# AU-Master-Thesis/magics

Hardware: AMD Instinct MI355X
Metric: GBP iterations/sec (whole node), N robots x K horizon (higher is better)
Workload: dtype f64

## Files before the change

### magics_amd/csrc/mgx_dev.h

```cpp
#pragma once
#include <cstdint>

namespace mgx {

constexpr int SNAP_W = 24;

struct BlobLayout {
    int K, E1;
    __host__ __device__ constexpr BlobLayout(int k) : K(k), E1(4 * k - 6 + 1) {}
    __host__ __device__ constexpr int prior() const { return 0; }
    __host__ __device__ constexpr int bel() const { return 20 * K; }
    __host__ __device__ constexpr int cov() const { return 40 * K; }
    __host__ __device__ constexpr int mu() const { return 56 * K; }
    __host__ __device__ constexpr int fv() const { return 60 * K; }
    __host__ __device__ constexpr int valid() const { return 60 * K + 20 * E1; }
    __host__ __device__ constexpr int inout_words() const { return 16 * K + 4 * K + 20 * E1 + K; }
    __host__ __device__ constexpr int words() const { return 61 * K + 20 * E1; }
};

struct IrEdgeRec {
    int32_t src_var;
    int32_t src_robot;
    uint32_t created;
    int32_t dst;
// ... 183 lines not shown

constexpr int MAX_SEGS = 32;

struct LingerPlan {
    uint32_t n, has_upd;
    uint32_t ext[MAX_SEGS / 4], n_int[MAX_SEGS / 4];
    double upd_max_speed, upd_delta_t;
    unsigned long long number;
};
constexpr int LINGER_PLAN_DWORDS = (int)(sizeof(LingerPlan) / 4);
constexpr unsigned LINGER_SLOT_HEAD = 128u, LINGER_UPD_BYTES = 48u;
static_assert(LINGER_PLAN_DWORDS == 24, "eight chunks of three dwords");
struct LingerBox {
    unsigned long long posted;
    unsigned long long close_req;
    unsigned long long taken;
    unsigned long long reserved;
    unsigned long long closed;
    unsigned long long pad[3];
    LingerPlan plan[2];
};

struct SweepRan {
    int32_t variant = 0;
    int32_t ir_mode = -1;
};

struct SegPlan {
    int32_t n;
    uint8_t ext[MAX_SEGS];
    uint8_t n_int[MAX_SEGS];
    unsigned long long flag_base;
    long long timeout_ticks;
    unsigned long long launch_seq;
    long long census_ticks;
    unsigned long long agree_seq;
    long long linger_ticks;
    const LingerBox *linger_box;
    const double *linger_upd;
    unsigned long long linger_upd_stride;
    unsigned char *linger_dev;
    unsigned long long linger_dev_stride;
    unsigned long long *linger_go;
};
constexpr unsigned RESIDENT_GO = 1u, RESIDENT_ABORT = 2u;

constexpr int AGREE_LOOK = 0, AGREE_SIGN_IN = 1, AGREE_ABORT = 2;
constexpr int AGREE_HISTORY = 6;
constexpr unsigned AGREE_LOST = 3u;
__device__ inline unsigned agree_on_launch(unsigned long long *word, unsigned long long L, unsigned n_ranks, int action) {
    constexpr unsigned long long HMASK = (1ull << (2 * AGREE_HISTORY)) - 1ull;
    unsigned long long declined = 0ull;
    for (int i = 0; i < AGREE_HISTORY; i++) declined |= (unsigned long long)RESIDENT_ABORT << (2 * i);
    unsigned long long cur = __hip_atomic_load(word, __ATOMIC_RELAXED, __HIP_MEMORY_SCOPE_SYSTEM);
    for (;;) {
        const unsigned long long cl = cur >> 28, hist = (cur >> 16) & HMASK;
        const unsigned st = (unsigned)(cur >> 14) & 3u, cnt = (unsigned)cur & 0x3fffu;
        if (cl == L && st) return st;
        if (cl > L) {
            const unsigned long long back = cl - L;
            if (back > (unsigned long long)AGREE_HISTORY) return AGREE_LOST;
            const unsigned was = (unsigned)(hist >> (2 * (back - 1ull))) & 3u;
            return was ? was : AGREE_LOST;
        }
        if (action == AGREE_LOOK) return 0u;
        unsigned long long h = hist;
// ... 23 lines not shown
```

### magics_amd/csrc/mgx_sweep.h

```cpp
#pragma once
#include <hip/hip_runtime.h>

#include "gbp_math.h"
#include "mgx_dev.h"

namespace mgx {

constexpr int SWEEP_BLOCK = 128;
enum { ROLE_DYN = 0, ROLE_UV = 1 };
#ifndef MGX_WIDE
#define MGX_WIDE 0
#endif
template <int KT, bool PERSIST>
constexpr int sweep_waves() { return (MGX_WIDE && PERSIST && KT > 0 && 4 * KT <= 64) ? 4 : 2; }
template <int KT, bool PERSIST>
constexpr int sweep_threads() { return 64 * sweep_waves<KT, PERSIST>(); }

__device__ __forceinline__ void ld_soa4(const double *base, int stride, int item, double (&o)[4]) {
#pragma unroll
    for (int c = 0; c < 4; c++) o[c] = base[(size_t)c * stride + item];
}
__device__ __forceinline__ void ld_soa16(const double *base, int stride, int item, double (&o)[16]) {
#pragma unroll
    for (int c = 0; c < 16; c++) o[c] = base[(size_t)c * stride + item];
// ... 412 lines not shown
        const int a2 = 2 * slot, b2 = 2 * (1 - slot);
        const int it = r * (K - 1) + f;
#pragma unroll
        for (int i = 0; i < 2; i++)
#pragma unroll
            for (int j = 0; j < 2; j++) {
                paa[i * 2 + j] = w.dyn_m[(size_t)((a2 + i) * 4 + (a2 + j)) * w.ND + it];
                pab[i * 2 + j] = w.dyn_m[(size_t)((a2 + i) * 4 + (b2 + j)) * w.ND + it];
                pba[i * 2 + j] = w.dyn_m[(size_t)((b2 + i) * 4 + (a2 + j)) * w.ND + it];
                pbb[i * 2 + j] = w.dyn_m[(size_t)((b2 + i) * 4 + (b2 + j)) * w.ND + it];
            }
    };
    if (is_dyn) {
        const int f = lane % (K - 1), slot = lane / (K - 1);
        if (!PERSIST) load_dyn_potential(maa, mab, mba, mbb);
        dyn_other_var = f + 1 - slot;
        dyn_other_edge = (1 - slot) * (K - 1) + f;
    }
    const bool obs_rows = (4 * (K - 2) <= 64) && !(w.enable & 8u);
    const int uvar = (is_trk ? lane - (K - 2) : lane) + 1;
    const int uedge = n_dyn + lane;
    int trk_rec = 0;
    float trk_lp[2] = {0.f, 0.f};
    double trk_lv = 0.0;
    const int trk_item = r * (K - 2) + (uvar - 1);
    if (is_trk) {
        trk_rec = w.trk_record[trk_item];
        trk_lp[0] = w.trk_last_pos[trk_item];
        trk_lp[1] = w.trk_last_pos[(size_t)w.NT + trk_item];
        trk_lv = w.trk_last_val[trk_item];
    }

    const bool do_extf = !PERSIST && HAS_IR && (ext_mask & PH_EXT_FACTOR) && radio && ir_on;
    bool pf_on = false, pf_present = false;
    MGX_EDGE_REGS(pf_er);
    double pf_bmu[4] = {0.0, 0.0, 0.0, 0.0}, pf_rec[SNAP_W];
#pragma unroll
    for (int c = 0; c < SNAP_W; c++) pf_rec[c] = 0.0;
    uint8_t pf_gate = 0;
    int pf_dst = 0;
    const int n_in = (PERSIST && K > 1) ? ne / (K - 1) : 0;
    auto edge_of_lane = [&](int q) __attribute__((always_inline)) {
        if (!PERSIST) return q;
        const int c = q / (K - 1);
        return (q - c * (K - 1)) * n_in + c;
    };
    int my_j = (HAS_IR && tid < ne) ? edge_of_lane(tid) : 0;
    if (HAS_IR && tid < ne) pf_gate = w.ir_gate[ie0 + my_j];
    if (do_extf && tid < ne) {
        MGX_EDGE_LOAD(pf_er, &w.ir_rec[ie0 + my_j]);
        pf_dst = pf_er_dst;
        ld_soa4(w.ir_bmu, w.NI, ie0 + my_j, pf_bmu);
    }
    if (PERSIST && tid < ne) {
        MGX_EDGE_LOAD(pf_er, &w.ir_rec[ie0 + my_j]);
        pf_dst = pf_er_dst;
    }
    auto quad_gather = [&](auto fetch, unsigned ro_mine, double (&out)[SNAP_W]) __attribute__((always_inline)) {
        v4u32 R[4][3];
#pragma unroll
        for (int s4 = 0; s4 < 4; s4++) {
            unsigned rb;
            if (s4 == 0) rb = (unsigned)__builtin_amdgcn_mov_dpp((int)ro_mine, 0x00, 0xf, 0xf, true);
            else if (s4 == 1) rb = (unsigned)__builtin_amdgcn_mov_dpp((int)ro_mine, 0x55, 0xf, 0xf, true);
            else if (s4 == 2) rb = (unsigned)__builtin_amdgcn_mov_dpp((int)ro_mine, 0xAA, 0xf, 0xf, true);
            else rb = (unsigned)__builtin_amdgcn_mov_dpp((int)ro_mine, 0xFF, 0xf, 0xf, true);
#pragma unroll
            for (int t3 = 0; t3 < 3; t3++) R[s4][t3] = fetch(rb + 64u * t3 + 16u * (unsigned)(lane & 3));
        }
#pragma unroll
        for (int t3 = 0; t3 < 3; t3++) {
            unsigned dw[4][4];
#pragma unroll
            for (int wd = 0; wd < 4; wd++) {
                unsigned x[4] = {R[0][t3][wd], R[1][t3][wd], R[2][t3][wd], R[3][t3][wd]};
                quad_transpose4(x, lane);
#pragma unroll
                for (int v = 0; v < 4; v++) dw[wd][v] = x[v];
            }
#pragma unroll
            for (int v = 0; v < 4; v++) {
                out[2 * (4 * t3 + v)] = __hiloint2double((int)dw[1][v], (int)dw[0][v]);
                out[2 * (4 * t3 + v) + 1] = __hiloint2double((int)dw[3][v], (int)dw[2][v]);
            }
        }
    };
    auto fetch_plain = [&](unsigned off) __attribute__((always_inline)) {
        return *reinterpret_cast<const v4u32 *>(reinterpret_cast<const char *>(w.snap[w.cur]) + off);
    };
    uint32_t r_epoch = 0;
    int r_irp[3] = {0, 0, 0};
    if (tid < K) {
        r_epoch = w.snap_epoch[w.cur][v0 + tid];
        if (HAS_IR) {
            r_irp[0] = w.ir_var_ptr[v0 + tid];
            r_irp[1] = w.ir_var_mid[v0 + tid];
            r_irp[2] = w.ir_var_ptr[v0 + tid + 1];
        }
    }
    double u_rec[4] = {0.0, 0.0, 0.0, 0.0}, u_bel = 0.0;
    if (w.upd) {
#pragma unroll
        for (int c = 0; c < 4; c++) u_rec[c] = w.upd[(size_t)r * 4 + c];
        if (lane < 20 && role < 2) u_bel = blob[L.bel() + lane * K + (role == 0 ? K - 1 : 0)];
    }
    const bool recompute = (PERSIST ? plan.ext[0] != 0 : (ext_mask & PH_EXT_FACTOR) != 0) && radio && ir_on;
    double r_ir[6] = {0.0, 0.0, 0.0, 0.0, 0.0, 0.0};
    bool r_ir_on = false;

    auto chain_second_link = [&]() {
        if (STAGE_IR && tid < ne && !(recompute && pf_gate == 1)) {
            const size_t e = (size_t)(ie0 + my_j);
            r_ir_on = true;
            r_ir[0] = w.ir_fv_eta[0 * (size_t)w.NI + e];
            r_ir[1] = w.ir_fv_eta[1 * (size_t)w.NI + e];
            r_ir[2] = w.ir_fv_lam[0 * (size_t)w.NI + e];
            r_ir[3] = w.ir_fv_lam[1 * (size_t)w.NI + e];
            r_ir[4] = w.ir_fv_lam[4 * (size_t)w.NI + e];
            r_ir[5] = w.ir_fv_lam[5 * (size_t)w.NI + e];
        }
        if (do_extf) {
            pf_on = tid < ne && pf_gate == 1;
            if (pf_on) pf_present = w.snap_epoch[w.cur][pf_er_src_var] > pf_er_created;
            quad_gather(fetch_plain, pf_on ? (unsigned)pf_er_src_var * (unsigned)(SNAP_W * sizeof(double)) : 0u, pf_rec);
        }
    };
    unsigned long long early_decision = 0ull;
    {
        const double *src = w.snap[w.cur] + (size_t)v0 * SNAP_W;
        if constexpr (KT > 0) {
            StageRegs<20 * KT, NT> r_prior;
            StageRegs<BlobLayout(KT).inout_words() - 16 * KT, NT> r_io;
            constexpr int IT = (SNAP_W * KT + NT - 1) / NT;
            double r_snap[IT];
            r_prior.load(blob + L.prior(), tid);
            r_io.load(blob + L.mu(), tid);
#pragma unroll
            for (int it = 0; it < IT; it++) {
                const int t = tid + it * NT;
                r_snap[it] = (t < SNAP_W * K) ? src[t] : 0.0;
            }
            chain_second_link();
            if (census && BIG && tid == 0) early_decision = __hip_atomic_load(cold().decision, __ATOMIC_RELAXED, __HIP_MEMORY_SCOPE_AGENT);
            r_prior.store(s_prior, tid);
            r_io.store(s_mu, tid);
#pragma unroll
            for (int it = 0; it < IT; it++) {
                const int t = tid + it * NT;
                if (t < SNAP_W * K) s_snap[(t % SNAP_W) * K + (t / SNAP_W)] = r_snap[it];
            }
        } else {
            copy_words(s_prior, blob + L.prior(), 20 * K, tid, NT);
            chain_second_link();
            if (census && BIG && tid == 0) early_decision = __hip_atomic_load(cold().decision, __ATOMIC_RELAXED, __HIP_MEMORY_SCOPE_AGENT);
            copy_words(s_mu, blob + L.mu(), L.inout_words() - 16 * K, tid, NT);
            for (int t = tid; t < SNAP_W * K; t += NT) s_snap[(t % SNAP_W) * K + (t / SNAP_W)] = src[t];
// ... 41 lines not shown
                v = __hip_atomic_load(cold().decision, __ATOMIC_RELAXED, __HIP_MEMORY_SCOPE_AGENT);
                if ((v >> 2) != seq && wall_clock64() - t0 > 4 * cold_plan().census_ticks) {
                    if (SHARD && cold_plan().agree_seq != 0ull) {
                        const unsigned a = agree_on_launch(cold().agree, cold_plan().agree_seq, (unsigned)cold().n_ranks, AGREE_ABORT);
                        if (a == RESIDENT_GO) continue;
                        if (a == AGREE_LOST) __hip_atomic_store(cold().sweep_err, cold_plan().agree_seq, __ATOMIC_RELAXED, __HIP_MEMORY_SCOPE_SYSTEM);
                    }
                    if (__hip_atomic_compare_exchange_strong(cold().decision, &v, seq * 4ull + RESIDENT_ABORT, __ATOMIC_RELAXED, __ATOMIC_RELAXED,
                                                             __HIP_MEMORY_SCOPE_AGENT)) {
                        __hip_atomic_store(cold().decision_host, seq * 4ull + RESIDENT_ABORT, __ATOMIC_RELAXED, __HIP_MEMORY_SCOPE_SYSTEM);
                        v = seq * 4ull + RESIDENT_ABORT;
                    }
                }
            }
            abort_launch = (v & 3ull) == RESIDENT_ABORT ? 1 : 0;
        }
        return __syncthreads_or(abort_launch) != 0;
    };
    if (census && CENSUS_EARLY && census_says_abort(early_decision)) return;
    if (PLDS && w.upd) {
        if (tid < 4) s_urec[tid] = tid == 0 ? u_rec[0] : (tid == 1 ? u_rec[1] : (tid == 2 ? u_rec[2] : u_rec[3]));
        if (lane < 20 && role < 2) s_tmp[4 * K + role * 20 + lane] = u_bel;
        __syncthreads();
    }
    uint32_t my_epoch = 0u;
    STAMP(t_staged);

    const int VL = w.R_local * K;
    const unsigned xrec_bytes = PERSIST ? (unsigned)VL * (unsigned)XREC_BYTES : 0u;
    const __amdgpu_buffer_rsrc_t rs_x = sc1_rsrc(PERSIST ? w.xrec[0] : nullptr, 2u * xrec_bytes);
    constexpr unsigned GHOST_BIT = 0x80000000u;
    const unsigned gx_bytes = SHARD ? (unsigned)(w.V - VL) * (unsigned)XREC_BYTES : 0u;
    const __amdgpu_buffer_rsrc_t rs_gx = sc1_rsrc(SHARD ? w.gxrec[0] : nullptr, 2u * gx_bytes);
    auto gather_records = [&](auto fetch, bool mine, unsigned off_mine, uint32_t seq, double (&out)[SNAP_W], uint32_t &deliveries) __attribute__((always_inline)) {
        v4u32 R[XREC_CHUNKS];
        const unsigned cstride = 16u * (unsigned)K;
#pragma unroll
        for (int ch = 0; ch < XREC_CHUNKS; ch++) R[ch] = v4u32{0u, 0u, 0u, 0u};
        const bool remote = SHARD && (off_mine & GHOST_BIT) != 0u;
        const bool any_remote = SHARD && __ballot(remote) != 0ull;
        if (mine) {
#pragma unroll
            for (int ch = 0; ch < XREC_CHUNKS; ch++) R[ch] = fetch(off_mine + (unsigned)ch * cstride);
        }
        if constexpr (SHARD) {
            if (any_remote) {
#pragma unroll
                for (int ch = 0; ch < XREC_CHUNKS; ch++) R[ch].w ^= remote ? xrec_mix(R[ch].x, R[ch].y, R[ch].z) : 0u;
            }
        }
        auto word_of = [&](const v4u32 &c) __attribute__((always_inline)) { return c.w; };
        long long t0 = 0;
        for (unsigned spins = 0;; spins++) {
            bool missing = false;
#pragma unroll
            for (int ch = 0; ch < XREC_CHUNKS; ch++) missing = missing || word_of(R[ch]) != seq;
            missing = missing && mine;
            if (__ballot(missing) == 0ull) break;
#ifdef MGX_POLL_SLEEP
            __builtin_amdgcn_s_sleep(MGX_POLL_SLEEP);
#else
            __builtin_amdgcn_s_sleep(32);
#endif
            if (spins == 0u) t0 = wall_clock64();
            if ((spins & 31u) == 31u) {
                bool stop = __hip_atomic_load(cold().sweep_abort, __ATOMIC_RELAXED, __HIP_MEMORY_SCOPE_AGENT) != 0ull;
                if (!stop && wall_clock64() - t0 > cold_plan().timeout_ticks) {
                    __hip_atomic_store(cold().sweep_abort, (unsigned long long)seq, __ATOMIC_RELAXED, __HIP_MEMORY_SCOPE_AGENT);
                    __hip_atomic_store(cold().sweep_err, (unsigned long long)seq, __ATOMIC_RELAXED, __HIP_MEMORY_SCOPE_SYSTEM);
                    stop = true;
                }
                if (__ballot(stop) != 0ull) break;
            }
            if (missing) {
                unsigned again = 0u;
#pragma unroll
                for (int ch = 0; ch < XREC_CHUNKS; ch++)
                    if (word_of(R[ch]) != seq) { again |= 1u << ch; R[ch] = fetch(off_mine + (unsigned)ch * cstride); }
                if constexpr (SHARD) {
                    if (remote) {
#pragma unroll
                        for (int ch = 0; ch < XREC_CHUNKS; ch++)
                            if ((again >> ch) & 1u) R[ch].w ^= xrec_mix(R[ch].x, R[ch].y, R[ch].z);
                    }
                }
            }
        }
        auto D = [&](int n) __attribute__((always_inline)) { return R[n / 3][n % 3]; };
#pragma unroll
        for (int n = 0; n < 22; n++) out[n] = __hiloint2double((int)D(2 * n + 1), (int)D(2 * n));
        out[22] = 0.0;
        out[23] = 0.0;
        deliveries = D(XREC_EPOCH_DWORD);
#ifdef MGX_XREC_CHECKSUM
        if (mine) {
            unsigned x = 0u;
#pragma unroll
            for (int n = 0; n < XREC_PAYLOAD_DWORDS; n++) x ^= D(n);
            const unsigned o = off_mine & 0x7fffffffu, rob = o / ((unsigned)K * (unsigned)XREC_BYTES);
            const unsigned want_id = rob * 64u + (o - rob * (unsigned)K * (unsigned)XREC_BYTES) / 16u;
            if (x != R[15].x || R[15].y != want_id)
                __hip_atomic_store(cold().sweep_err, 0xBAD0000000000000ull | ((unsigned long long)(R[15].y & 0xfffffu) << 28) | ((unsigned long long)(want_id & 0xfffffu) << 8) | (seq & 0xffu),
                                   __ATOMIC_RELAXED, __HIP_MEMORY_SCOPE_SYSTEM);
        }
#endif
    };
    double *s_xmu = s_tmp;
    bool have_xmu = false;
#ifdef MGX_STAMPS
    unsigned long long q_arrive = 0ull, t_edges0 = 0ull;
    unsigned long long *tl = (PERSIST && w.dbg) ? w.dbg + (size_t)(w.R_local + 4) * 48 + (size_t)r * 64 : nullptr;
#define TLSTAMP(kk, what) do { if (tl && role == ROLE_UV && lane == 0 && (kk) >= 0 && (kk) < 16) tl[(kk) * 4 + (what)] = __builtin_amdgcn_s_memrealtime(); } while (0)
#else
#define TLSTAMP(kk, what)
#endif
    auto external_factor_sweep = [&](int k, int kg, bool store_fv) __attribute__((always_inline)) {
        const int buf = PERSIST ? ((w.cur + kg) & 1) : w.cur;
#ifdef MGX_STAMPS
        t_edges0 = __builtin_readcyclecounter();
#endif
        if (radio && ir_on) {
            auto fetch_xrec = [&](unsigned off) __attribute__((always_inline)) {
                if constexpr (SHARD) {
                    if (off & GHOST_BIT) return ld16_system_raw(rs_gx, off & ~GHOST_BIT, buf ? gx_bytes : 0u);
                }
                return ld16_agent_raw(rs_x, off, buf ? xrec_bytes : 0u);
            };
            const uint32_t want_seq = xrec_seq(plan.flag_base + (unsigned long long)kg);
            for (int j0 = 0; j0 < ne; j0 += NT) {
                const int q = j0 + tid;
                const int j = j0 == 0 ? my_j : (q < ne ? edge_of_lane(q) : 0);
                const int e = ie0 + j;
                MGX_EDGE_REGS(er);
                double ao_eta[4], ao_lam[16], a_mu[4], b_mu[4];
                bool a_present;
                double grec[SNAP_W];
                uint32_t grec_deliveries = 0u;
                bool mine = false;
                if (PERSIST || j0 > 0) {
                    if (j0 == 0) {
                        mine = tid < ne && pf_gate == 1;
                        if (mine) MGX_EDGE_COPY(er, pf_er);
                    } else if (j0 > 0 && q < ne && w.ir_gate[e] == 1) {
                        mine = true;
                        MGX_EDGE_LOAD(er, &w.ir_rec[e]);
                    }
                    if (PERSIST && k > 0) {
                        const bool ghost_src = SHARD && mine && er_src_var >= VL;
                        const int sv = mine ? (ghost_src ? er_src_var - VL : er_src_var) : 0, si = sv % K;
                        const unsigned off_mine = ((unsigned)(sv - si) * (unsigned)XREC_BYTES + 16u * (unsigned)si) | (ghost_src ? GHOST_BIT : 0u);
                        if (j0 == 0) TLSTAMP(k - 1, 2);
                        gather_records(fetch_xrec, mine, off_mine, want_seq, grec, grec_deliveries);
                        if (j0 == 0) TLSTAMP(k - 1, 3);
                        DELAY_AT(4, j0 == 0);
                        DELAY_AT(6, j0 == 0 && role == ROLE_UV);
                        DELAY_AT(7, j0 == 0 && role == ROLE_DYN);
                    } else {
                        quad_gather(fetch_plain, mine ? (unsigned)er_src_var * (unsigned)(SNAP_W * sizeof(double)) : 0u, grec);
                    }
                    if (!mine) continue;
                }

                if (PERSIST) {
                    if (have_xmu) {
                        const int i = er_dst & 0xffff;
#pragma unroll
                        for (int c = 0; c < 4; c++) b_mu[c] = s_xmu[c * K + i];
                    } else {
                        ld_soa4(w.ir_bmu, w.NI, e, b_mu);
                    }
                    if (j0 == 0 && pf_present) {
                        a_present = true;
                    } else {
                        if (k > 0) a_present = grec_deliveries > er_created;
                        else a_present = w.snap_epoch[buf][er_src_var] > er_created;
                        if (j0 == 0) pf_present = a_present;
                    }
#ifdef MGX_STAMPS
                    asm volatile("s_waitcnt vmcnt(0)" ::: "memory");
                    if (j0 == 0) { const unsigned long long _n = __builtin_readcyclecounter(); q_arrive += _n - t_edges0; }
#endif
#pragma unroll
                    for (int c = 0; c < 4; c++) ao_eta[c] = grec[c];
#pragma unroll
                    for (int c = 0; c < 16; c++) ao_lam[c] = grec[4 + c];
#pragma unroll
                    for (int c = 0; c < 4; c++) a_mu[c] = grec[20 + c];
                } else if (j0 == 0) {
                    if (q >= ne) continue;
                    if (!pf_on) continue;
                    MGX_EDGE_COPY(er, pf_er);
                    a_present = pf_present;
#pragma unroll
                    for (int c = 0; c < 4; c++) b_mu[c] = pf_bmu[c];
#pragma unroll
                    for (int c = 0; c < 4; c++) ao_eta[c] = pf_rec[c];
#pragma unroll
                    for (int c = 0; c < 16; c++) ao_lam[c] = pf_rec[4 + c];
#pragma unroll
                    for (int c = 0; c < 4; c++) a_mu[c] = pf_rec[20 + c];
                } else {
                    ld_soa4(w.ir_bmu, w.NI, e, b_mu);
                    a_present = w.snap_epoch[w.cur][er_src_var] > er_created;
#pragma unroll
                    for (int c = 0; c < 4; c++) ao_eta[c] = grec[c];
#pragma unroll
                    for (int c = 0; c < 16; c++) ao_lam[c] = grec[4 + c];
#pragma unroll
                    for (int c = 0; c < 4; c++) a_mu[c] = grec[20 + c];
                }
                if (!a_present) {
#pragma unroll
                    for (int c = 0; c < 4; c++) { ao_eta[c] = 0.0; a_mu[c] = 0.0; }
#pragma unroll
                    for (int c = 0; c < 16; c++) ao_lam[c] = 0.0;
                }
                const int dslot = er_dst >> 16;
                double x_lo[4], x_hi[4], o6[6];
#pragma unroll
                for (int c = 0; c < 4; c++) {
                    x_lo[c] = dslot ? a_mu[c] : b_mu[c];
                    x_hi[c] = dslot ? b_mu[c] : a_mu[c];
                }
                const bool live_msg = interrobot_message_compact(x_lo, x_hi, er_d_safe, er_inv_d_safe, er_offset, w.inv_s2_ir, dslot, ao_eta, ao_lam, o6);
                if (!live_msg) {
#pragma unroll
                    for (int c = 0; c < 6; c++) o6[c] = 0.0;
                }
#ifdef MGX_STAMPS
                if (tl && k == 5 && j0 == 0 && role < 2) {
                    const unsigned long long lv = __ballot(live_msg);
                    if (lane == __ffsll((unsigned long long)__ballot(true)) - 1) {
                        tl[60 + role] = (unsigned long long)__popcll(lv);
                        if (role == ROLE_UV) {
                            unsigned hw, xcc;
                            asm volatile("s_getreg_b32 %0, hwreg(HW_REG_HW_ID)" : "=s"(hw));
                            asm volatile("s_getreg_b32 %0, hwreg(HW_REG_XCC_ID)" : "=s"(xcc));
                            tl[62] = ((unsigned long long)xcc << 32) | hw;
                        }
                    }
                }
#endif
                if (store_fv && !(STAGE_IR && (hints & HINT_IR_DEAD))) {
                    w.ir_fv_eta[0 * (size_t)w.NI + e] = o6[0];
                    w.ir_fv_eta[1 * (size_t)w.NI + e] = o6[1];
                    w.ir_fv_lam[0 * (size_t)w.NI + e] = o6[2];
                    w.ir_fv_lam[1 * (size_t)w.NI + e] = o6[3];
                    w.ir_fv_lam[4 * (size_t)w.NI + e] = o6[4];
                    w.ir_fv_lam[5 * (size_t)w.NI + e] = o6[5];
                }
                if (STAGE_IR) {
                    double *p = s_ir + j * IR_STRIDE;
#pragma unroll
                    for (int c = 0; c < 6; c++) p[c] = o6[c];
                }
            }
        }
// ... 399 lines not shown
            s_fv[c * E1 + e] = s_sh[c * E1 + e];
        }
    };
    int last_int_seg = -1, last_ext_seg = -1;
    int kbase = 0;
    if (PLDS && lane == 0) s_ps[0] = 0u;
    if (PLDS) __builtin_amdgcn_wave_barrier();
#ifdef MGX_STAMPS
    unsigned long long c_f = 0, c_fb = 0, c_v = 0, c_vb = 0, t_extf = t_staged, t_extv = t_staged, t_loop0 = t_staged;
    unsigned long long rt0 = __builtin_amdgcn_s_memrealtime();
    unsigned long long p_wait = 0, p_extf = 0, p_extv = 0, p_int = 0, p_pub = 0;
    unsigned long long qs[16] = {0, 0, 0, 0, 0, 0, 0, 0, 0, 0, 0, 0, 0, 0, 0, 0};
#define PSTAMP(v) const unsigned long long v = __builtin_readcyclecounter()
#define QSTAMP(i, since) do { const unsigned long long _n = __builtin_readcyclecounter(); qs[i] += _n - (since); (since) = _n; } while (0)
#define QBEGIN(v) unsigned long long v = __builtin_readcyclecounter()
#else
#define PSTAMP(v)
#define QSTAMP(i, since)
#define QBEGIN(v)
#endif
    for (int k = 0; PLDS || k < nseg; k++) {
        if (k == 0) {
            const int plans_done = PLDS ? (int)ps_word(0) : 0;
            const bool upd_now = PLDS ? plan_dword(1) != 0u : w.upd != nullptr;
            if (upd_now) {
                if constexpr (PLDS) {
#pragma unroll
                    for (int c = 0; c < 4; c++) u_rec[c] = s_urec[c];
                    u_bel = (lane < 20 && role < 2) ? s_tmp[4 * K + role * 20 + lane] : 0.0;
                }
                const double upd_max_speed = PLDS ? reinterpret_cast<const double *>(s_plan + 2 + MAX_SEGS / 2)[0] : w.upd_max_speed;
                const double upd_delta_t = PLDS ? reinterpret_cast<const double *>(s_plan + 2 + MAX_SEGS / 2)[1] : w.upd_delta_t;
                const uint32_t what = (uint32_t)u_rec[3];
                const int i = role == 0 ? K - 1 : 0;
                if (role < 2 && (role == 0 ? (what & 1u) : (what & 2u))) {
                    double m[4];
                    if (role == 0) {
                        const double ex = s_mu[0 * K + i], ey = s_mu[1 * K + i];
                        double hx = u_rec[0] - ex, hy = u_rec[1] - ey;
                        const double dist = std::sqrt(hx * hx + hy * hy);
                        double nx = hx, ny = hy;
                        if (!(dist == 0.0 || std::isinf(dist))) { nx = hx / dist; ny = hy / dist; }
                        const double sp = (upd_max_speed < dist || dist != dist) ? upd_max_speed : dist;
                        const double vx = sp * nx, vy = sp * ny;
                        m[0] = ex + vx * upd_delta_t; m[1] = ey + vy * upd_delta_t; m[2] = vx; m[3] = vy;
                    } else {
        #pragma unroll
                        for (int c = 0; c < 4; c++) {
                            const double m0 = s_mu[c * K + 0], m1 = s_mu[c * K + 1];
                            m[c] = m0 + u_rec[2] * (m1 - m0);
                        }
                    }
                    __builtin_amdgcn_wave_barrier();
                    if (lane < 4) {
                        double pl[4];
        #pragma unroll
                        for (int c = 0; c < 4; c++) pl[c] = s_prior[(4 + lane * 4 + c) * K + i];
                        const double pe = ((pl[0] * m[0] + pl[1] * m[1]) + pl[2] * m[2]) + pl[3] * m[3];
                        s_prior[lane * K + i] = pe;
                        blob[L.prior() + lane * K + i] = pe;
                    } else if (lane < 8) {
                        const double mc = lane == 4 ? m[0] : (lane == 5 ? m[1] : (lane == 6 ? m[2] : m[3]));
                        s_mu[(lane - 4) * K + i] = mc;
                        s_snap[(20 + lane - 4) * K + i] = mc;
                        if (PERSIST && have_xmu) s_xmu[(lane - 4) * K + i] = mc;
                    } else if (lane == 8) {
                        s_epoch[i] += 1;
// ... 145 lines not shown
                if (role == ROLE_UV && lane < 4 * K) {
                    double mu_fin = mu_i;
                    const int xs = s_xok[i];
                    if (!(ok_i && fin_i)) {
                        mu_fin = s_xmu[q * K + i];
                        if (!ok_i && (xs & 1)) {
#pragma unroll
                            for (int j = 0; j < 4; j++) s_cov[(j * 4 + q) * K + i] = s_tmp[(4 + j * 4 + q) * K + i];
                        }
                    }
                    s_mu[q * K + i] = mu_fin;
                    s_snap[(20 + q) * K + i] = mu_fin;
                    if (is_last) {
                        s_prior[q * K + i] = s_snap[q * K + i];
#pragma unroll
                        for (int c = 0; c < 4; c++) s_prior[(4 + q * 4 + c) * K + i] = s_snap[(4 + q * 4 + c) * K + i];
                    }
                    if (q == 0) {
                        if (ok_i) {
                            s_valid[i] = fin_i ? 1 : 0;
                            s_covset[i] = 1;
                        } else if (xs & 1) {
                            s_valid[i] = (xs & 2) ? 1 : 0;
                            s_covset[i] = 1;
                        }
                    }
                }
                if (ir_on && (!is_last_ext_seg || lingers)) have_xmu = true;
                if (ir_on && is_last_ext_seg) {
                    for (int q = tid; q < ne; q += NT) {
                        const int e = ie0 + (q == tid ? my_j : edge_of_lane(q));
                        int dst;
                        if (q == tid) {
                            if (!pf_gate) continue;
                            dst = pf_dst;
                        } else {
                            if (!w.ir_gate[e]) continue;
                            dst = w.ir_rec[e].dst;
                        }
                        const int iv = dst & 0xffff;
#pragma unroll
                        for (int c = 0; c < 4; c++) w.ir_bmu[(size_t)c * w.NI + e] = s_xmu[c * K + iv];
                    }
                }
                if (is_last) __syncthreads();
                itf += 1;
                early = false;
            } else if ((ext_k & PH_EXT_VARIABLE) && radio) {
                const bool ext_is_last = last_seg && n_int_k == 0;
                double *s_sum = ext_is_last ? s_prior : s_tmp;
                prefired = !early && n_int_k > 0 && !idle && (int_k & PH_INT_FACTOR) && skip0 == 0u;
                const bool keep_means = ir_on && (!is_last_ext_seg || lingers);
                if (role == ROLE_UV) {
                    variable_sums(s_sum, false, false);
                    QSTAMP(4, qt);
                    finish(s_sum, false);
                    if (keep_means && lane < 4 * K) s_xmu[lane] = s_mu[lane] - 0.0;
                }
                if (prefired && (NW == 4 || role == ROLE_UV)) unary_messages(0u, s_sh, itf);
                if (prefired && is_dyn && (w.enable & 1u)) dynamic_messages(s_sh);
                QSTAMP(6, qt);
                if (keep_means) have_xmu = true;
                if (ir_on && is_last_ext_seg) {
                    __syncthreads();
                    for (int q = tid; q < ne; q += NT) {
                        const int e = ie0 + (q == tid ? my_j : edge_of_lane(q));
                        int dst;
                        if (q == tid) {
                            if (!pf_gate) continue;
                            dst = pf_dst;
                        } else {
                            if (!w.ir_gate[e]) continue;
                            dst = w.ir_rec[e].dst;
                        }
                        const int i = dst & 0xffff;
#pragma unroll
                        for (int c = 0; c < 4; c++) w.ir_bmu[(size_t)c * w.NI + e] = s_mu[c * K + i] - 0.0;
                    }
                }
                if (prefired) __syncthreads();
            }
            if (early || prefired) {
                double *t_ = s_fv;
                s_fv = s_sh;
                s_sh = t_;
            }
        } else if (ext_k & PH_EXT_VARIABLE) {
            const bool ext_is_last = PERSIST ? (last_seg && n_int_k == 0) : !has_int_var;
            double *s_sum = ext_is_last ? s_prior : s_tmp;
            if (radio) variable_sums(s_sum, false, false);
            QSTAMP(4, qt);
            __syncthreads();
            QSTAMP(5, qt);
            prefired = !early && radio && n_int_k > 0 && !idle && (int_k & PH_INT_FACTOR) && skip0 == 0u;
            if (prefired && is_dyn && (w.enable & 1u)) dynamic_messages(s_fv);
            if (PERSIST && early && radio && role == ROLE_DYN) adopt_early(lane, 64);
            if (radio && is_var) variable_finish(s_sum, false);
            if (prefired) unary_messages(0u, s_fv, itf);
            QSTAMP(6, qt);
            __syncthreads();
            QSTAMP(7, qt);
            if (PERSIST && radio && ir_on && (!is_last_ext_seg || lingers)) {
                if (tid < 4 * K) s_xmu[tid] = s_mu[tid] - 0.0;
                have_xmu = true;
            }
            if (radio && ir_on && (!PERSIST || is_last_ext_seg)) {
                for (int q = tid; q < ne; q += NT) {
                    const int e = ie0 + (q == tid ? my_j : edge_of_lane(q));
                    int dst;
                    if (q == tid && (do_extf || PERSIST)) {
                        if (!pf_gate) continue;
                        dst = pf_dst;
                    } else {
                        if (!w.ir_gate[e]) continue;
                        dst = w.ir_rec[e].dst;
                    }
                    const int i = dst & 0xffff;
#pragma unroll
                    for (int c = 0; c < 4; c++) w.ir_bmu[(size_t)c * w.NI + e] = s_mu[c * K + i] - 0.0;
                }
            }
        }
        QSTAMP(8, qt);
        PSTAMP(ps3);
#ifdef MGX_STAMPS
        if (k == 0) { t_extv = __builtin_readcyclecounter(); t_loop0 = t_extv; rt0 = __builtin_amdgcn_s_memrealtime(); }
#endif
        if (PERSIST && !FUSED && early && !((ext_k & PH_EXT_VARIABLE) && radio)) {
            adopt_early(tid, NT);
            __syncthreads();
        }
        if (PERSIST && early) prefired = true;
        early = false;
        for (int it = 0; it < n_int_k && !idle && !par_done; it++) {
            asm volatile("" : "+v"(tid), "+v"(lane));
            STAMP(t0);
            if ((int_k & PH_INT_FACTOR) && it == 0 && prefired) {
                itf += 1;
            } else if (int_k & PH_INT_FACTOR) {
                if (is_dyn && (w.enable & 1u) && !(it == 0 && (skip0 & 1u))) dynamic_messages(s_fv);
                if (pending) {
                    finish(s_snap, true);
                    if (NW == 4) __syncthreads();
                }
// ... 231 lines not shown
```

### magics_amd/csrc/mgx_world_launch.inc

```
static int direct_exchange(mgx_world *w);
static int rccl_exchange(mgx_world *w);
static int sweep(mgx_world *w, int32_t robot, uint32_t ext_mask, uint32_t int_mask, int n_int, uint32_t hints = 0);
static void log_launch(mgx_world *w, int robot, uint32_t ext_mask, uint32_t int_mask, int n_int);

static void log_plan(mgx_world *w, const std::vector<Launch> &plan, size_t from = 0, size_t n = ~(size_t)0) {
    for (size_t k = from; k < plan.size() && k - from < n; k++) log_launch(w, -1, plan[k].ext, int_phases(plan[k]), plan[k].n_int);
}
static int run_segments(mgx_world *w, const std::vector<Launch> &plan, size_t from, const RidingUpdates &upd) {
    for (size_t k = from; k < plan.size(); k++) {
        const bool rides = k == from && upd.dev;
        if (rides) { w->d.upd = upd.dev; w->d.upd_max_speed = upd.max_speed; w->d.upd_delta_t = upd.delta_t; }
        int rc = sweep(w, -1, plan[k].ext, int_phases(plan[k]), plan[k].n_int, plan[k].hints);
        w->d.upd = nullptr;
        if (rides && upd.slot >= 0) {
            const hipError_t e = w->stage.release(upd.slot, w->stream);
            if (rc == MGX_OK && e != hipSuccess) rc = fail(MGX_ERR_HIP, "event record: %s", hipGetErrorString(e));
        }
        if (rc != MGX_OK) return rc;
    }
    return MGX_OK;
}
template <class F>
static int spin_until(F done) {
    const double t0 = StageTimer::now();
// ... 404 lines not shown
    un.before = standing(w);
    un.upd = RidingUpdates{};
    if (upd.any()) {
        double *slot = linger_upd_slot(w, P);
        if (upd.host != slot) memcpy(slot, upd.host, 4 * (size_t)w->d.R_local * sizeof(double));
        un.upd.host = slot;
        un.upd.max_speed = upd.max_speed;
        un.upd.delta_t = upd.delta_t;
    }
    __atomic_store_n(&lg.box()->posted, P, __ATOMIC_RELEASE);
    stand_at(w, un.before.after_post((int)plan.size()));
    w->stale_kinds |= ~w->p.enable_mask & 15u;
    w->last_sweep_launches++;
    w->last_sweep = lg.ran;
    w->last_sweep_form = MGX_SWEEP_FORM_POSTED;
}

static int post_into_open_launch(mgx_world *w, const std::vector<Launch> &plan) {
    if (!w->res.linger.open) return 0;
    if (!w->res.riding.postable()) {
        const int rc = linger_close(w);
        return rc != MGX_OK ? rc : 0;
    }
    const int r = linger_prepare_post(w, plan);
    if (r == 1) linger_post(w, plan, w->res.riding);
    return r;
}
static int part_plan(mgx_world *w, const std::vector<Launch> &plan, size_t i0, bool sharded, bool census, bool ranks_agree, bool lingers, SegPlan &sp) {
    ResidentLaunches &rl = w->res;
    sp = SegPlan{};
    sp.n = fill_segments(plan, i0, sp.ext, sp.n_int);
    sp.flag_base = rl.flag_base;
    sp.timeout_ticks = ResidentKnobs::timeout_ticks();
    if (census) {
        sp.launch_seq = ++rl.launch_seq;
        sp.census_ticks = sharded ? ResidentKnobs::census_ticks_sharded() : ResidentKnobs::census_ticks();
        if (ranks_agree) sp.agree_seq = ++w->xres.agree_seq;
    }
    if (lingers) {
        const int rc = ensure_linger_box(w);
        if (rc != MGX_OK) return rc;
        void *bd = nullptr;
        HIP_TRY(hipHostGetDevicePointer(&bd, rl.linger.box(), 0));
        sp.linger_ticks = linger_ticks(w);
        sp.linger_box = (const LingerBox *)bd;
        sp.linger_upd = reinterpret_cast<const double *>(reinterpret_cast<const char *>(bd) + sizeof(LingerBox));
        sp.linger_upd_stride = (unsigned long long)rl.linger.upd_stride;
        sp.linger_dev = rl.linger.dev.p;
        sp.linger_dev_stride = (unsigned long long)rl.linger.dev_stride;
        sp.linger_go = rl.linger.go.p;
    }
    return MGX_OK;
}
static void part_launched(mgx_world *w, const std::vector<Launch> &plan, size_t i0, const SegPlan &sp, const RidingUpdates &rode, bool can, bool sharded,
                          const SweepRan &ran) {
    ResidentLaunches &rl = w->res;
    w->last_sweep_launches++;
    rl.launches++;
    if (can) {
        w->last_sweep = ran;
        w->last_sweep_form = sharded ? MGX_SWEEP_FORM_SHARDED : MGX_SWEEP_FORM_RESIDENT;
    }
    if (sp.linger_ticks > 0) {
        ResidentLaunches::Linger &lg = rl.linger;
        lg.open = true;
        lg.seq0 = sp.launch_seq;
// ... 79 lines not shown
```

### magics_amd/csrc/mgx_world_types.h

```cpp
#pragma once
#include <hip/hip_runtime.h>

#include <algorithm>
#include <cmath>
#include <cstdarg>
#include <cstdio>
#include <cstdlib>
#include <dlfcn.h>
#include <cstring>
#include <map>
#include <memory>
#include <string>
#include <utility>
#include <vector>

#include "../../include/mgx.h"
#include "gbp_math.h"
#include "mgx_dev.h"
#include "mgx_grid.h"
#include "mgx_search.h"
#include "mgx_resident.h"

namespace mgx {
size_t sweep_lds_bytes(int K, int ir_edges);
// ... 372 lines not shown
    MappedBlock &operator=(const MappedBlock &) = delete;
    ~MappedBlock() { release(); }
    void release() { if (p) (void)hipHostFree(p); p = nullptr; }
    hipError_t alloc(size_t bytes) {
        release();
        const hipError_t e = hipHostMalloc(&p, bytes, hipHostMallocMapped);
        if (e == hipSuccess) memset(p, 0, bytes);
        return e;
    }
};

struct Submitted {
    bool active = false;
    unsigned long long number = 0;
    std::vector<Launch> plan;
    Standing before;
    bool partial = false;
    RidingUpdates upd;
    void take_back(mgx_world *w);
};

struct ResidentLaunches {
    DevBuf<unsigned long long> sweep_flag_buf, sweep_abort_buf, census_buf, decision_buf;
    DevBuf<unsigned char> xrec_buf;
    MappedBlock decision_mem;
    unsigned long long *decision_host() const { return (unsigned long long *)decision_mem.p; }
    DevBuf<int32_t> peer_ptr_dev, peer_ptr_dev_b;
    size_t peer_idx_off = 0;
    std::vector<int32_t> peer_fill;
    bool peers_valid = false;
    unsigned long long flag_base = 0;
    unsigned long long launch_seq = 0;
    enum Mode : int32_t { OFF = 0, ON = 1, DECLINE = 2 } mode = ON;
    Backoff backoff;
    int cap = -1, cap_sharded = -1;
    int capacity_for(const DevWorld &d, bool sharded) {
        int &c = sharded ? cap_sharded : cap;
        if (c < 0) c = sweep_resident_capacity(d, sharded);
        return c;
    }
    uint64_t aborts = 0, launches = 0;
    Submitted pending;
    RidingUpdates riding;
    struct Linger {
        long long ticks = -1;
        MappedBlock box_mem;
        LingerBox *box() const { return (LingerBox *)box_mem.p; }
        size_t upd_stride = 0;
        DevBuf<unsigned long long> go;
        DevBuf<unsigned char> dev;
        size_t dev_stride = 0;
        bool open = false, hold = false;
        unsigned long long seq0 = 0;
        SweepRan ran;
        uint32_t taken_in_launch = 0;
        int useless = 0;
        uint32_t streak = 0;
        Submitted un;
        uint64_t launches = 0, posts = 0, reruns = 0, ended_by_device = 0;
    } linger;
    void arrays_rebuilt() {
        peers_valid = false;
        sweep_flag_buf.n = 0;
        flag_base = 0;
        cap = cap_sharded = -1;
    }
// ... 279 lines not shown
```

Baseline: 126,100.

## Gather only probe chunks of inter-robot records when factor is far

In the persistent sweep, gather_records first fetches and polls only the two chunks holding the source position means and delivery count. The remaining chunks are fetched only when the factor is live, that is, when the source lies within d_safe of the destination mean, or when the previous iteration judged it near within a configurable margin (MGX_GATHER_MARGIN, default 2x). This cuts cross-device record traffic and polling for distant robot pairs. In exchange it adds a second polling round for near factors, zeroes messages built from partial records, and moves the b_mu load earlier.

```diff
diff --git a/magics_amd/csrc/mgx_dev.h b/magics_amd/csrc/mgx_dev.h
--- a/magics_amd/csrc/mgx_dev.h
+++ b/magics_amd/csrc/mgx_dev.h
@@ -239,6 +239,7 @@
     uint8_t n_int[MAX_SEGS];
     unsigned long long flag_base;
     long long timeout_ticks;
+    double gather_margin;
     unsigned long long launch_seq;
     long long census_ticks;
     unsigned long long agree_seq;
diff --git a/magics_amd/csrc/mgx_sweep.h b/magics_amd/csrc/mgx_sweep.h
--- a/magics_amd/csrc/mgx_sweep.h
+++ b/magics_amd/csrc/mgx_sweep.h
@@ -468,12 +468,13 @@
     }
 
     const bool do_extf = !PERSIST && HAS_IR && (ext_mask & PH_EXT_FACTOR) && radio && ir_on;
-    bool pf_on = false, pf_present = false;
+    bool pf_on = false;
+    constexpr unsigned PF_GATE = 0xffu, PF_PRESENT = 0x100u, PF_NEAR = 0x200u;
+    unsigned pf_flags = PF_NEAR;
     MGX_EDGE_REGS(pf_er);
     double pf_bmu[4] = {0.0, 0.0, 0.0, 0.0}, pf_rec[SNAP_W];
 #pragma unroll
     for (int c = 0; c < SNAP_W; c++) pf_rec[c] = 0.0;
-    uint8_t pf_gate = 0;
     int pf_dst = 0;
     const int n_in = (PERSIST && K > 1) ? ne / (K - 1) : 0;
     auto edge_of_lane = [&](int q) __attribute__((always_inline)) {
@@ -482,7 +483,7 @@
         return (q - c * (K - 1)) * n_in + c;
     };
     int my_j = (HAS_IR && tid < ne) ? edge_of_lane(tid) : 0;
-    if (HAS_IR && tid < ne) pf_gate = w.ir_gate[ie0 + my_j];
+    if (HAS_IR && tid < ne) pf_flags |= w.ir_gate[ie0 + my_j];
     if (do_extf && tid < ne) {
         MGX_EDGE_LOAD(pf_er, &w.ir_rec[ie0 + my_j]);
         pf_dst = pf_er_dst;
@@ -545,7 +546,7 @@
     bool r_ir_on = false;
 
     auto chain_second_link = [&]() {
-        if (STAGE_IR && tid < ne && !(recompute && pf_gate == 1)) {
+        if (STAGE_IR && tid < ne && !(recompute && (pf_flags & PF_GATE) == 1u)) {
             const size_t e = (size_t)(ie0 + my_j);
             r_ir_on = true;
             r_ir[0] = w.ir_fv_eta[0 * (size_t)w.NI + e];
@@ -556,8 +557,8 @@
             r_ir[5] = w.ir_fv_lam[5 * (size_t)w.NI + e];
         }
         if (do_extf) {
-            pf_on = tid < ne && pf_gate == 1;
-            if (pf_on) pf_present = w.snap_epoch[w.cur][pf_er_src_var] > pf_er_created;
+            pf_on = tid < ne && (pf_flags & PF_GATE) == 1u;
+            if (pf_on && w.snap_epoch[w.cur][pf_er_src_var] > pf_er_created) pf_flags |= PF_PRESENT;
             quad_gather(fetch_plain, pf_on ? (unsigned)pf_er_src_var * (unsigned)(SNAP_W * sizeof(double)) : 0u, pf_rec);
         }
     };
@@ -665,61 +666,101 @@
     constexpr unsigned GHOST_BIT = 0x80000000u;
     const unsigned gx_bytes = SHARD ? (unsigned)(w.V - VL) * (unsigned)XREC_BYTES : 0u;
     const __amdgpu_buffer_rsrc_t rs_gx = sc1_rsrc(SHARD ? w.gxrec[0] : nullptr, 2u * gx_bytes);
-    auto gather_records = [&](auto fetch, bool mine, unsigned off_mine, uint32_t seq, double (&out)[SNAP_W], uint32_t &deliveries) __attribute__((always_inline)) {
+    constexpr int XREC_PROBE = 13;
+    static_assert(XREC_EPOCH_DWORD / 3 == XREC_PROBE + 1 && 40 / 3 == XREC_PROBE && 43 / 3 == XREC_PROBE + 1 && XREC_PROBE + 1 < XREC_CHUNKS,
+                  "the probe — the two position means (payload dwords 40..43) and the delivery count — is chunks 13 and 14");
+    auto gather_records = [&](auto fetch, bool mine, bool full, auto live, unsigned off_mine, uint32_t seq, double (&out)[SNAP_W], uint32_t &deliveries,
+                              bool &whole) __attribute__((always_inline)) {
         v4u32 R[XREC_CHUNKS];
         const unsigned cstride = 16u * (unsigned)K;
+        auto in_probe = [](int ch) constexpr { return ch == XREC_PROBE || ch == XREC_PROBE + 1; };
 #pragma unroll
         for (int ch = 0; ch < XREC_CHUNKS; ch++) R[ch] = v4u32{0u, 0u, 0u, 0u};
+#ifdef MGX_XREC_CHECKSUM
+        full = true;
+#endif
         const bool remote = SHARD && (off_mine & GHOST_BIT) != 0u;
         const bool any_remote = SHARD && __ballot(remote) != 0ull;
+        bool rest = mine && full;
         if (mine) {
 #pragma unroll
-            for (int ch = 0; ch < XREC_CHUNKS; ch++) R[ch] = fetch(off_mine + (unsigned)ch * cstride);
+            for (int ch = 0; ch < XREC_CHUNKS; ch++)
+                if (in_probe(ch)) R[ch] = fetch(off_mine + (unsigned)ch * cstride);
+            if (rest) {
+#pragma unroll
+                for (int ch = 0; ch < XREC_CHUNKS; ch++)
+                    if (!in_probe(ch)) R[ch] = fetch(off_mine + (unsigned)ch * cstride);
+            }
         }
         if constexpr (SHARD) {
             if (any_remote) {
 #pragma unroll
-                for (int ch = 0; ch < XREC_CHUNKS; ch++) R[ch].w ^= remote ? xrec_mix(R[ch].x, R[ch].y, R[ch].z) : 0u;
+                for (int ch = 0; ch < XREC_CHUNKS; ch++) R[ch].w ^= (remote && (in_probe(ch) || rest)) ? xrec_mix(R[ch].x, R[ch].y, R[ch].z) : 0u;
             }
         }
         auto word_of = [&](const v4u32 &c) __attribute__((always_inline)) { return c.w; };
+        auto D = [&](int n) __attribute__((always_inline)) { return R[n / 3][n % 3]; };
         long long t0 = 0;
-        for (unsigned spins = 0;; spins++) {
-            bool missing = false;
-#pragma unroll
-            for (int ch = 0; ch < XREC_CHUNKS; ch++) missing = missing || word_of(R[ch]) != seq;
-            missing = missing && mine;
-            if (__ballot(missing) == 0ull) break;
+        bool stop_all = false;
+        auto poll = [&](bool polled, auto watched) __attribute__((always_inline)) {
+            for (unsigned spins = 0;; spins++) {
+                bool missing = false;
+#pragma unroll
+                for (int ch = 0; ch < XREC_CHUNKS; ch++)
+                    if (watched(ch)) missing = missing || word_of(R[ch]) != seq;
+                missing = missing && polled;
+                if (__ballot(missing) == 0ull) break;
 #ifdef MGX_POLL_SLEEP
-            __builtin_amdgcn_s_sleep(MGX_POLL_SLEEP);
+                __builtin_amdgcn_s_sleep(MGX_POLL_SLEEP);
 #else
-            __builtin_amdgcn_s_sleep(32);
+                __builtin_amdgcn_s_sleep(32);
 #endif
-            if (spins == 0u) t0 = wall_clock64();
-            if ((spins & 31u) == 31u) {
-                bool stop = __hip_atomic_load(cold().sweep_abort, __ATOMIC_RELAXED, __HIP_MEMORY_SCOPE_AGENT) != 0ull;
-                if (!stop && wall_clock64() - t0 > cold_plan().timeout_ticks) {
-                    __hip_atomic_store(cold().sweep_abort, (unsigned long long)seq, __ATOMIC_RELAXED, __HIP_MEMORY_SCOPE_AGENT);
-                    __hip_atomic_store(cold().sweep_err, (unsigned long long)seq, __ATOMIC_RELAXED, __HIP_MEMORY_SCOPE_SYSTEM);
-                    stop = true;
-                }
-                if (__ballot(stop) != 0ull) break;
-            }
-            if (missing) {
-                unsigned again = 0u;
+                if (spins == 0u) t0 = wall_clock64();
+                if ((spins & 31u) == 31u) {
+                    bool stop = __hip_atomic_load(cold().sweep_abort, __ATOMIC_RELAXED, __HIP_MEMORY_SCOPE_AGENT) != 0ull;
+                    if (!stop && wall_clock64() - t0 > cold_plan().timeout_ticks) {
+                        __hip_atomic_store(cold().sweep_abort, (unsigned long long)seq, __ATOMIC_RELAXED, __HIP_MEMORY_SCOPE_AGENT);
+                        __hip_atomic_store(cold().sweep_err, (unsigned long long)seq, __ATOMIC_RELAXED, __HIP_MEMORY_SCOPE_SYSTEM);
+                        stop = true;
+                    }
+                    if (__ballot(stop) != 0ull) { stop_all = true; break; }
+                }
+                if (missing) {
+                    unsigned again = 0u;
+#pragma unroll
+                    for (int ch = 0; ch < XREC_CHUNKS; ch++)
+                        if (watched(ch) && word_of(R[ch]) != seq) { again |= 1u << ch; R[ch] = fetch(off_mine + (unsigned)ch * cstride); }
+                    if constexpr (SHARD) {
+                        if (remote) {
+#pragma unroll
+                            for (int ch = 0; ch < XREC_CHUNKS; ch++)
+                                if ((again >> ch) & 1u) R[ch].w ^= xrec_mix(R[ch].x, R[ch].y, R[ch].z);
+                        }
+                    }
+                }
+            }
+        };
+        poll(mine, [&](int ch) __attribute__((always_inline)) { return in_probe(ch) || rest; });
+        const bool is_live = live(__hiloint2double((int)D(41), (int)D(40)), __hiloint2double((int)D(43), (int)D(42)), D(XREC_EPOCH_DWORD));
+        const bool more = mine && !rest && is_live;
+        if (__ballot(more) != 0ull && !stop_all) {
+            if (more) {
 #pragma unroll
                 for (int ch = 0; ch < XREC_CHUNKS; ch++)
-                    if (word_of(R[ch]) != seq) { again |= 1u << ch; R[ch] = fetch(off_mine + (unsigned)ch * cstride); }
-                if constexpr (SHARD) {
-                    if (remote) {
-#pragma unroll
-                        for (int ch = 0; ch < XREC_CHUNKS; ch++)
-                            if ((again >> ch) & 1u) R[ch].w ^= xrec_mix(R[ch].x, R[ch].y, R[ch].z);
-                    }
-                }
-            }
-        }
-        auto D = [&](int n) __attribute__((always_inline)) { return R[n / 3][n % 3]; };
+                    if (!in_probe(ch)) R[ch] = fetch(off_mine + (unsigned)ch * cstride);
+            }
+            if constexpr (SHARD) {
+                if (more && remote) {
+#pragma unroll
+                    for (int ch = 0; ch < XREC_CHUNKS; ch++)
+                        if (!in_probe(ch)) R[ch].w ^= xrec_mix(R[ch].x, R[ch].y, R[ch].z);
+                }
+            }
+            poll(more, [&](int ch) __attribute__((always_inline)) { return !in_probe(ch); });
+        }
+        rest = rest || more;
+        whole = rest;
+        if (!rest) R[XREC_PROBE].x = 0u;
 #pragma unroll
         for (int n = 0; n < 22; n++) out[n] = __hiloint2double((int)D(2 * n + 1), (int)D(2 * n));
         out[22] = 0.0;
@@ -765,25 +806,40 @@
                 const int j = j0 == 0 ? my_j : (q < ne ? edge_of_lane(q) : 0);
                 const int e = ie0 + j;
                 MGX_EDGE_REGS(er);
-                double ao_eta[4], ao_lam[16], a_mu[4], b_mu[4];
+                double ao_eta[4], ao_lam[16], a_mu[4], b_mu[4] = {0.0, 0.0, 0.0, 0.0};
                 bool a_present;
                 double grec[SNAP_W];
                 uint32_t grec_deliveries = 0u;
+                bool grec_whole = true;
                 bool mine = false;
                 if (PERSIST || j0 > 0) {
                     if (j0 == 0) {
-                        mine = tid < ne && pf_gate == 1;
+                        mine = tid < ne && (pf_flags & PF_GATE) == 1u;
                         if (mine) MGX_EDGE_COPY(er, pf_er);
                     } else if (j0 > 0 && q < ne && w.ir_gate[e] == 1) {
                         mine = true;
                         MGX_EDGE_LOAD(er, &w.ir_rec[e]);
+                    }
+                    if (PERSIST && mine) {
+                        if (have_xmu) {
+                            const int i = er_dst & 0xffff;
+#pragma unroll
+                            for (int c = 0; c < 4; c++) b_mu[c] = s_xmu[c * K + i];
+                        } else {
+                            ld_soa4(w.ir_bmu, w.NI, e, b_mu);
+                        }
                     }
                     if (PERSIST && k > 0) {
                         const bool ghost_src = SHARD && mine && er_src_var >= VL;
                         const int sv = mine ? (ghost_src ? er_src_var - VL : er_src_var) : 0, si = sv % K;
                         const unsigned off_mine = ((unsigned)(sv - si) * (unsigned)XREC_BYTES + 16u * (unsigned)si) | (ghost_src ? GHOST_BIT : 0u);
                         if (j0 == 0) TLSTAMP(k - 1, 2);
-                        gather_records(fetch_xrec, mine, off_mine, want_seq, grec, grec_deliveries);
+                        auto factor_is_live = [&](double ax, double ay, uint32_t deliveries) __attribute__((always_inline)) {
+                            const bool present = (j0 == 0 && (pf_flags & PF_PRESENT) != 0u) || deliveries > er_created;
+                            const double dx = (present ? ax : 0.0) - b_mu[0], dy = (present ? ay : 0.0) - b_mu[1];
+                            return !(dx * dx + dy * dy >= er_d_safe * er_d_safe);
+                        };
+                        gather_records(fetch_xrec, mine, j0 > 0 || (pf_flags & PF_NEAR) != 0u, factor_is_live, off_mine, want_seq, grec, grec_deliveries, grec_whole);
                         if (j0 == 0) TLSTAMP(k - 1, 3);
                         DELAY_AT(4, j0 == 0);
                         DELAY_AT(6, j0 == 0 && role == ROLE_UV);
@@ -795,19 +851,12 @@
                 }
 
                 if (PERSIST) {
-                    if (have_xmu) {
-                        const int i = er_dst & 0xffff;
-#pragma unroll
-                        for (int c = 0; c < 4; c++) b_mu[c] = s_xmu[c * K + i];
-                    } else {
-                        ld_soa4(w.ir_bmu, w.NI, e, b_mu);
-                    }
-                    if (j0 == 0 && pf_present) {
+                    if (j0 == 0 && (pf_flags & PF_PRESENT) != 0u) {
                         a_present = true;
                     } else {
                         if (k > 0) a_present = grec_deliveries > er_created;
                         else a_present = w.snap_epoch[buf][er_src_var] > er_created;
-                        if (j0 == 0) pf_present = a_present;
+                        if (j0 == 0 && a_present) pf_flags |= PF_PRESENT;
                     }
 #ifdef MGX_STAMPS
                     asm volatile("s_waitcnt vmcnt(0)" ::: "memory");
@@ -819,11 +868,16 @@
                     for (int c = 0; c < 16; c++) ao_lam[c] = grec[4 + c];
 #pragma unroll
                     for (int c = 0; c < 4; c++) a_mu[c] = grec[20 + c];
+                    if (j0 == 0) {
+                        const double dx = (a_present ? a_mu[0] : 0.0) - b_mu[0], dy = (a_present ? a_mu[1] : 0.0) - b_mu[1];
+                        const bool far = dx * dx + dy * dy >= cold_plan().gather_margin * (er_d_safe * er_d_safe);
+                        pf_flags = far ? (pf_flags & ~PF_NEAR) : (pf_flags | PF_NEAR);
+                    }
                 } else if (j0 == 0) {
                     if (q >= ne) continue;
                     if (!pf_on) continue;
                     MGX_EDGE_COPY(er, pf_er);
-                    a_present = pf_present;
+                    a_present = (pf_flags & PF_PRESENT) != 0u;
 #pragma unroll
                     for (int c = 0; c < 4; c++) b_mu[c] = pf_bmu[c];
 #pragma unroll
@@ -855,7 +909,7 @@
                     x_lo[c] = dslot ? a_mu[c] : b_mu[c];
                     x_hi[c] = dslot ? b_mu[c] : a_mu[c];
                 }
-                const bool live_msg = interrobot_message_compact(x_lo, x_hi, er_d_safe, er_inv_d_safe, er_offset, w.inv_s2_ir, dslot, ao_eta, ao_lam, o6);
+                const bool live_msg = interrobot_message_compact(x_lo, x_hi, er_d_safe, er_inv_d_safe, er_offset, w.inv_s2_ir, dslot, ao_eta, ao_lam, o6) && grec_whole;
                 if (!live_msg) {
 #pragma unroll
                     for (int c = 0; c < 6; c++) o6[c] = 0.0;
@@ -1321,7 +1375,8 @@
                 const double upd_max_speed = PLDS ? reinterpret_cast<const double *>(s_plan + 2 + MAX_SEGS / 2)[0] : w.upd_max_speed;
                 const double upd_delta_t = PLDS ? reinterpret_cast<const double *>(s_plan + 2 + MAX_SEGS / 2)[1] : w.upd_delta_t;
                 const uint32_t what = (uint32_t)u_rec[3];
-                const int i = role == 0 ? K - 1 : 0;
+                int i = role == 0 ? K - 1 : 0;
+                asm volatile("" : "+v"(i));
                 if (role < 2 && (role == 0 ? (what & 1u) : (what & 2u))) {
                     double m[4];
                     if (role == 0) {
@@ -1533,7 +1588,7 @@
                         const int e = ie0 + (q == tid ? my_j : edge_of_lane(q));
                         int dst;
                         if (q == tid) {
-                            if (!pf_gate) continue;
+                            if (!(pf_flags & PF_GATE)) continue;
                             dst = pf_dst;
                         } else {
                             if (!w.ir_gate[e]) continue;
@@ -1568,7 +1623,7 @@
                         const int e = ie0 + (q == tid ? my_j : edge_of_lane(q));
                         int dst;
                         if (q == tid) {
-                            if (!pf_gate) continue;
+                            if (!(pf_flags & PF_GATE)) continue;
                             dst = pf_dst;
                         } else {
                             if (!w.ir_gate[e]) continue;
@@ -1610,7 +1665,7 @@
                     const int e = ie0 + (q == tid ? my_j : edge_of_lane(q));
                     int dst;
                     if (q == tid && (do_extf || PERSIST)) {
-                        if (!pf_gate) continue;
+                        if (!(pf_flags & PF_GATE)) continue;
                         dst = pf_dst;
                     } else {
                         if (!w.ir_gate[e]) continue;
diff --git a/magics_amd/csrc/mgx_world_launch.inc b/magics_amd/csrc/mgx_world_launch.inc
--- a/magics_amd/csrc/mgx_world_launch.inc
+++ b/magics_amd/csrc/mgx_world_launch.inc
@@ -460,6 +460,7 @@
     sp.n = fill_segments(plan, i0, sp.ext, sp.n_int);
     sp.flag_base = rl.flag_base;
     sp.timeout_ticks = ResidentKnobs::timeout_ticks();
+    sp.gather_margin = rl.gather_margin;
     if (census) {
         sp.launch_seq = ++rl.launch_seq;
         sp.census_ticks = sharded ? ResidentKnobs::census_ticks_sharded() : ResidentKnobs::census_ticks();
diff --git a/magics_amd/csrc/mgx_world_types.h b/magics_amd/csrc/mgx_world_types.h
--- a/magics_amd/csrc/mgx_world_types.h
+++ b/magics_amd/csrc/mgx_world_types.h
@@ -428,6 +428,13 @@
     unsigned long long flag_base = 0;
     unsigned long long launch_seq = 0;
     enum Mode : int32_t { OFF = 0, ON = 1, DECLINE = 2 } mode = ON;
+    static double gather_margin_from_env() {
+        const char *e = getenv("MGX_GATHER_MARGIN");
+        char *end = nullptr;
+        const double f = e ? strtod(e, &end) : 2.0;
+        return (e && (end == e || !(f >= 0.0))) ? 4.0 : f * f;
+    }
+    double gather_margin = gather_margin_from_env();
     Backoff backoff;
     int cap = -1, cap_sharded = -1;
     int capacity_for(const DevWorld &d, bool sharded) {
```

Result: slower. 119,600 (-5.1%).
